# SamsungLabs/nb-asr

Hardware: AMD Instinct MI355X
Metric: utterances_per_sec (higher is better)
Workload: dtype f32

## Files before the change

### nb_asr_amd/csrc/grouped_conv.hip

```cpp
#include "grouped_conv_impl.h"

namespace nbasr {

__global__ __launch_bounds__(256) void pack_grouped_weights_kernel(const float* __restrict__ w, float* __restrict__ wp,
                                                                   int channels, int cg, int k)
{
    const int n = channels * cg * k;
    for (int i = blockIdx.x * blockDim.x + threadIdx.x; i < n; i += gridDim.x * blockDim.x) {
        int e = i;
        const int co = e % cg; e /= cg;
        const int j = e % k; e /= k;
        const int ci = e % cg; e /= cg;
        const int g = e;
        wp[i] = w[((static_cast<size_t>(g) * cg + co) * cg + ci) * k + j];
    }
}

constexpr int SF_QUADS = 32, SF_FRAMES = 4 * SF_QUADS, SF_LANES = 8, SF_MAX_PER_LANE = 16;
__global__ __launch_bounds__(SF_QUADS * SF_LANES) void stats_finalize_kernel(const float* __restrict__ part, float* __restrict__ stats,
                                                                               int batch, int frames, int ld, int groups, int cg, int gpp, float eps)
{
    __shared__ float s_cnt[SF_LANES][SF_FRAMES], s_mean[SF_LANES][SF_FRAMES], s_m2[SF_LANES][SF_FRAMES];
    const int tq = threadIdx.x & (SF_QUADS - 1), pl = threadIdx.x / SF_QUADS;
    const int t0 = blockIdx.x * SF_FRAMES + 4 * tq;
    const int b = blockIdx.y;
    const int nparts = (groups + gpp - 1) / gpp;
    float cnt[4] = {0.f, 0.f, 0.f, 0.f}, mean[4] = {0.f, 0.f, 0.f, 0.f}, m2[4] = {0.f, 0.f, 0.f, 0.f};
    if (t0 < frames) {
        float4 pm[SF_MAX_PER_LANE], pq[SF_MAX_PER_LANE];
#pragma unroll
        for (int u = 0; u < SF_MAX_PER_LANE; ++u) {
            const int k = pl + u * SF_LANES;
            pm[u] = make_float4(0.f, 0.f, 0.f, 0.f); pq[u] = pm[u];
            if (k < nparts) {
                const float* prow = part + (static_cast<size_t>(k) * batch + b) * 2 * ld + t0;
                pm[u] = *reinterpret_cast<const float4*>(prow);
                pq[u] = *reinterpret_cast<const float4*>(prow + ld);
            }
        }
#pragma unroll
        for (int u = 0; u < SF_MAX_PER_LANE; ++u) {
            const int k = pl + u * SF_LANES;
            if (k < nparts) {
                const float nb = static_cast<float>(cg * min(gpp, groups - gpp * k));
                const float pmv[4] = {pm[u].x, pm[u].y, pm[u].z, pm[u].w}, pqv[4] = {pq[u].x, pq[u].y, pq[u].z, pq[u].w};
#pragma unroll
                for (int r = 0; r < 4; ++r) {
                    const float tot = cnt[r] + nb;
                    const float delta = pmv[r] - mean[r];
                    mean[r] += delta * (nb / tot);
                    m2[r] += pqv[r] + delta * delta * (cnt[r] * nb / tot);
                    cnt[r] = tot;
                }
            }
        }
    }
#pragma unroll
    for (int r = 0; r < 4; ++r) { s_cnt[pl][4 * tq + r] = cnt[r]; s_mean[pl][4 * tq + r] = mean[r]; s_m2[pl][4 * tq + r] = m2[r]; }
    __syncthreads();
    const int tf = threadIdx.x, t = blockIdx.x * SF_FRAMES + tf;
    if (tf >= SF_FRAMES || t >= ld) return;
    float* srow = stats + static_cast<size_t>(b) * 2 * ld;
    if (t >= frames) { srow[t] = 0.f; srow[ld + t] = 0.f; return; }
    float c = s_cnt[0][tf], mu = s_mean[0][tf], q = s_m2[0][tf];
#pragma unroll
    for (int p = 1; p < SF_LANES; ++p) {
        const float nb = s_cnt[p][tf];
        if (nb > 0.f) {
            const float tot = c + nb;
            const float delta = s_mean[p][tf] - mu;
            mu += delta * (nb / tot);
            q += s_m2[p][tf] + delta * delta * (c * nb / tot);
            c = tot;
        }
    }
    srow[t] = mu;
    srow[ld + t] = 1.0f / sqrtf(q / c + eps);
}

template <typename T>
__global__ __launch_bounds__(256) void skip_sum_kernel(
    const T* __restrict__ s0, const T* __restrict__ s1, const T* __restrict__ s2,
    T* __restrict__ y, size_t nchunks, int channels, int nq, const LnRef ln_s0)
{
    constexpr int FR = Chunk<T>::FR;
    const size_t stride = static_cast<size_t>(gridDim.x) * blockDim.x;
    for (size_t i = static_cast<size_t>(blockIdx.x) * blockDim.x + threadIdx.x; i < nchunks; i += stride) {
        float o[FR];
#pragma unroll
        for (int e = 0; e < FR; ++e) o[e] = 0.f;
        if (s0) {
            float v[FR];
            load_frames<FR>(s0 + i * FR, v);
            if (ln_s0.stats) {
                const size_t row = i / nq;
                const int q = static_cast<int>(i - row * nq);
                const int c = static_cast<int>(row % channels);
                const size_t b = row / channels;
                const float* mrow = ln_s0.stats + b * 2 * (static_cast<size_t>(nq) * FR);
                float m[FR], r[FR];
                load_frames<FR>(mrow + q * FR, m);
                load_frames<FR>(mrow + static_cast<size_t>(nq) * FR + q * FR, r);
                const float gam = ln_s0.gamma[c], bet = ln_s0.beta[c];
#pragma unroll
                for (int e = 0; e < FR; ++e) v[e] = ln_apply(v[e], m[e], r[e], gam, bet);
            }
#pragma unroll
            for (int e = 0; e < FR; ++e) o[e] += v[e];
        }
        if (s1) {
            float v[FR];
            load_frames<FR>(s1 + i * FR, v);
#pragma unroll
            for (int e = 0; e < FR; ++e) o[e] += v[e];
        }
        if (s2) {
            float v[FR];
            load_frames<FR>(s2 + i * FR, v);
#pragma unroll
            for (int e = 0; e < FR; ++e) o[e] += v[e];
        }
        store_frames<FR, false>(y + i * FR, o);
    }
}

template <typename E>
__global__ __launch_bounds__(256) void repitch_kernel(
    const E* __restrict__ src, E* __restrict__ dst, int rows, int frames, int ld_src, int ld_dst)
{
    const int t = blockIdx.x * blockDim.x + threadIdx.x;
    if (t >= ld_dst) return;
    for (int r = blockIdx.y; r < rows; r += gridDim.y)
        dst[static_cast<size_t>(r) * ld_dst + t] = (t < frames) ? src[static_cast<size_t>(r) * ld_src + t] : E(0);
}

template <int CG, int K, int D, bool LNX, bool STATS>
__global__ __launch_bounds__(256) void grouped_conv_f32_kernel(
    const float* __restrict__ x, const float* __restrict__ w, const float* __restrict__ bias,
    const float* __restrict__ s0, const float* __restrict__ s1, const float* __restrict__ s2,
    float* __restrict__ y, int channels, int frames, int ld, int groups, const LnRef ln_x, const LnRef ln_s0,
    float* __restrict__ part)
{
    constexpr int LPAD = pad_left(K, D, 1);
    constexpr int SPAN = (K - 1) * D;
    constexpr int QL = (LPAD + 3) / 4;
    constexpr int QR = (SPAN - LPAD + 3) / 4;
    constexpr int NCH = QL + 1 + QR;
    constexpr int BASE = 4 * QL - LPAD;

    const int nq = ld >> 2;
    const int lane = threadIdx.x & 63;
    const int wave = threadIdx.x >> 6;
    const int q = blockIdx.x * 64 + lane;
    const int g = __builtin_amdgcn_readfirstlane(blockIdx.y * 4 + wave);
    const int b = blockIdx.z;
    if (!STATS && g >= groups) return;
    const bool active = q < nq && g < groups;

    const int ga = g < groups ? g : groups - 1;
    const size_t row0 = (static_cast<size_t>(b) * channels + static_cast<size_t>(ga) * CG) * ld;
    const float* __restrict__ wg = w + static_cast<size_t>(ga) * (CG * CG * K);
    const float* __restrict__ bg = bias + ga * CG;

    float acc[CG][4];
#pragma unroll
    for (int co = 0; co < CG; ++co) {
        const float bv = bg[co];
#pragma unroll
        for (int r = 0; r < 4; ++r) acc[co][r] = bv;
    }

    typedef float f2 __attribute__((ext_vector_type(2)));
    constexpr int NP = LNX ? NCH * 2 : 1;
    f2 nmw[NP], rw[NP], kw[NP];
    if (LNX) {
        const float4* __restrict__ mrow = reinterpret_cast<const float4*>(ln_x.stats + static_cast<size_t>(b) * 2 * ld);
        const float4* __restrict__ rrow = mrow + nq;
#pragma unroll
        for (int c = 0; c < NCH; ++c) {
            const int qq = q - QL + c;
            float4 m = make_float4(0.f, 0.f, 0.f, 0.f), r = m;
            if (active && qq >= 0 && qq < nq) { m = mrow[qq]; r = rrow[qq]; }
            nmw[(2 * c) % NP] = f2{-m.x, -m.y}; nmw[(2 * c + 1) % NP] = f2{-m.z, -m.w};
            rw[(2 * c) % NP] = f2{r.x, r.y};    rw[(2 * c + 1) % NP] = f2{r.z, r.w};
            kw[(2 * c) % NP] = f2{r.x != 0.f ? 1.f : 0.f, r.y != 0.f ? 1.f : 0.f};
            kw[(2 * c + 1) % NP] = f2{r.z != 0.f ? 1.f : 0.f, r.w != 0.f ? 1.f : 0.f};
        }
    }

#pragma unroll 1
    for (int ci = 0; ci < CG; ++ci) {
        const float4* __restrict__ xrow = reinterpret_cast<const float4*>(x + row0 + static_cast<size_t>(ci) * ld);
        float xw[NCH * 4];
#pragma unroll
        for (int c = 0; c < NCH; ++c) {
            const int qq = q - QL + c;
            float4 v = make_float4(0.f, 0.f, 0.f, 0.f);
            if (active && qq >= 0 && qq < nq) v = xrow[qq];
            xw[4 * c + 0] = v.x; xw[4 * c + 1] = v.y; xw[4 * c + 2] = v.z; xw[4 * c + 3] = v.w;
        }
        if (LNX) {
            const float gam = ln_x.gamma[ga * CG + ci], bet = ln_x.beta[ga * CG + ci];
            const f2 gam2 = f2{gam, gam}, bet2 = f2{bet, bet};
#pragma unroll
            for (int p = 0; p < NCH * 2; ++p) {
                f2 v = f2{xw[2 * p], xw[2 * p + 1]};
                v = (v + nmw[p % NP]) * rw[p % NP];
                v = __builtin_elementwise_fma(v, gam2, bet2) * kw[p % NP];
                xw[2 * p] = v.x; xw[2 * p + 1] = v.y;
            }
        }
#pragma unroll
        for (int j = 0; j < K; ++j) {
#pragma unroll
            for (int co = 0; co < CG; ++co) {
                const float wv = wg[(co * CG + ci) * K + j];
#pragma unroll
                for (int r = 0; r < 4; ++r)
                    acc[co][r] = __builtin_fmaf(wv, xw[BASE + r + j * D], acc[co][r]);
            }
        }
    }

    if (!STATS && !active) return;
    const int t0 = q * 4;
    const bool ragged = __any(active && t0 + 3 >= frames) != 0;
    float4 sm = make_float4(0.f, 0.f, 0.f, 0.f), sr = sm;
    if (active && s0 && ln_s0.stats) {
        const float4* __restrict__ mrow = reinterpret_cast<const float4*>(ln_s0.stats + static_cast<size_t>(b) * 2 * ld);
        sm = mrow[q];
        sr = mrow[nq + q];
    }
    if (active) {
#pragma unroll
    for (int co = 0; co < CG; ++co) {
        const size_t off = row0 + static_cast<size_t>(co) * ld + t0;
        float o[4];
#pragma unroll
        for (int r = 0; r < 4; ++r) o[r] = relu_clamp(acc[co][r]);
        if (s0) {
            float4 v = *reinterpret_cast<const float4*>(s0 + off);
            if (ln_s0.stats) {
                const float gam = ln_s0.gamma[ga * CG + co], bet = ln_s0.beta[ga * CG + co];
                v.x = ln_apply(v.x, sm.x, sr.x, gam, bet); v.y = ln_apply(v.y, sm.y, sr.y, gam, bet);
                v.z = ln_apply(v.z, sm.z, sr.z, gam, bet); v.w = ln_apply(v.w, sm.w, sr.w, gam, bet);
            }
            o[0] += v.x; o[1] += v.y; o[2] += v.z; o[3] += v.w;
        }
        if (s1) { const float4 v = *reinterpret_cast<const float4*>(s1 + off); o[0] += v.x; o[1] += v.y; o[2] += v.z; o[3] += v.w; }
        if (s2) { const float4 v = *reinterpret_cast<const float4*>(s2 + off); o[0] += v.x; o[1] += v.y; o[2] += v.z; o[3] += v.w; }
        if (ragged) {
#pragma unroll
            for (int r = 0; r < 4; ++r) if (t0 + r >= frames) o[r] = 0.f;
        }
        typedef float f4v __attribute__((ext_vector_type(4)));
        __builtin_nontemporal_store(f4v{o[0], o[1], o[2], o[3]}, reinterpret_cast<f4v*>(y + off));
        if (STATS) {
#pragma unroll
            for (int r = 0; r < 4; ++r) acc[co][r] = o[r];
        }
    }
    }
    if (STATS) {
        __shared__ float sp[4][8][64];
        float pm[4], p2[4];
#pragma unroll
        for (int r = 0; r < 4; ++r) {
            float sum = 0.f;
#pragma unroll
            for (int co = 0; co < CG; ++co) sum += acc[co][r];
            pm[r] = sum * (1.0f / CG);
            float m2 = 0.f;
#pragma unroll
            for (int co = 0; co < CG; ++co) { const float d = acc[co][r] - pm[r]; m2 = __builtin_fmaf(d, d, m2); }
            p2[r] = m2;
        }
#pragma unroll
        for (int r = 0; r < 4; ++r) { sp[wave][r][lane] = pm[r]; sp[wave][4 + r][lane] = p2[r]; }
        __syncthreads();
        if (wave == 0 && q < nq) {
            const int g0 = blockIdx.y * 4;
            const int nw = min(4, groups - g0);
            float om[4], o2[4];
#pragma unroll
            for (int r = 0; r < 4; ++r) {
                float mean = 0.f;
                for (int k = 0; k < nw; ++k) mean += sp[k][r][lane];
                mean /= static_cast<float>(nw);
                float m2 = 0.f;
                for (int k = 0; k < nw; ++k) { const float d = sp[k][r][lane] - mean; m2 += sp[k][4 + r][lane] + CG * d * d; }
                om[r] = mean; o2[r] = m2;
            }
            float* prow = part + (static_cast<size_t>(blockIdx.y) * gridDim.z + b) * 2 * ld + t0;
            *reinterpret_cast<float4*>(prow) = make_float4(om[0], om[1], om[2], om[3]);
            *reinterpret_cast<float4*>(prow + ld) = make_float4(o2[0], o2[1], o2[2], o2[3]);
        }
    }
}

template <int CG, int K, int D>
static int launch_grouped_f32(const GroupedArgs<float>& a, hipStream_t stream)
{
    const int nq = a.ld / 4;
    dim3 grid((nq + 63) / 64, (a.groups + 3) / 4, a.batch);
#define NBASR_LAUNCH_GROUPED(LNX, STATS)                                                                                  \
    hipLaunchKernelGGL((grouped_conv_f32_kernel<CG, K, D, LNX, STATS>), grid, dim3(256), 0, stream, a.x, a.w, a.bias, a.s0, a.s1, \
                       a.s2, a.y, a.channels, a.frames, a.ld, a.groups, a.ln_x, a.ln_s0, a.part)
    if (a.ln_x.stats) { if (a.part) NBASR_LAUNCH_GROUPED(true, true); else NBASR_LAUNCH_GROUPED(true, false); }
    else              { if (a.part) NBASR_LAUNCH_GROUPED(false, true); else NBASR_LAUNCH_GROUPED(false, false); }
#undef NBASR_LAUNCH_GROUPED
    return launch_status("nbasr_grouped_conv1d_node");
}

template <int CG>
static int dispatch_kd_f32(int kernel, int dilation, const GroupedArgs<float>& a, hipStream_t stream)
{
    if (kernel == 5 && dilation == 1) return launch_grouped_f32<CG, 5, 1>(a, stream);
    if (kernel == 5 && dilation == 2) return launch_grouped_f32<CG, 5, 2>(a, stream);
    if (kernel == 7 && dilation == 1) return launch_grouped_f32<CG, 7, 1>(a, stream);
    if (kernel == 7 && dilation == 2) return launch_grouped_f32<CG, 7, 2>(a, stream);
    set_error("nbasr_grouped_conv1d_node: unsupported (kernel=%d, dilation=%d); search space has k in {5,7}, d in {1,2}", kernel, dilation);
    return NBASR_EINVAL;
}

int grouped_conv_f32_base(const GroupedArgs<float>& a, int kernel, int dilation, hipStream_t stream)
{
    switch (a.channels / a.groups) {
        case 6:  return dispatch_kd_f32<6>(kernel, dilation, a, stream);
        case 8:  return dispatch_kd_f32<8>(kernel, dilation, a, stream);
        case 10: return dispatch_kd_f32<10>(kernel, dilation, a, stream);
        case 12: return dispatch_kd_f32<12>(kernel, dilation, a, stream);
        default:
            set_error("nbasr_grouped_conv1d_node: channels/groups=%d unsupported (model widths give 6, 8, 10, 12)", a.channels / a.groups);
            return NBASR_EINVAL;
    }
}

}

using namespace nbasr;

extern "C" size_t nbasr_grouped_stats_workspace_bytes(int batch, int ld, int groups)
{
    if (batch <= 0 || ld <= 0 || groups <= 0) return 0;
    return static_cast<size_t>(groups) * batch * 2 * ld * sizeof(float);
}

static int grouped_node_impl(const char* what, const void* x, const float* w, const float* bias, const void* skip0, const void* skip1,
                             const void* skip2, void* y, int batch, int channels, int frames, int ld, int groups, int kernel,
                             int dilation, const nbasr_deferred_ln* ln, int ln_on_x, int ln_on_skip0, float* stats_ws, int dtype,
                             int variant, nbasr_stream_t stream)
{
    NBASR_REQUIRE(dtype == NBASR_F32 || dtype == NBASR_BF16, NBASR_EINVAL, "%s: dtype %d is neither NBASR_F32 nor NBASR_BF16", what, dtype);
    const bool alt2 = variant > 0 && (variant & ~(NBASR_GC_OSPLIT | NBASR_GC_PIPE)) == 0;
    const bool ring = variant == NBASR_GC_RING;
    NBASR_REQUIRE((variant >= 0 && variant <= (NBASR_GC_FPL8 | NBASR_GC_WPERM)) || ((alt2 || ring) && dtype == NBASR_F32), NBASR_EINVAL,
                  "%s: unknown variant %d (NBASR_GC_OSPLIT / NBASR_GC_PIPE / NBASR_GC_RING: fp32 only, not with the other bits)", what, variant);
    NBASR_REQUIRE(aligned16(stats_ws), NBASR_EALIGN, "%s: statistics buffers must be 16-byte aligned", what);
    NBASR_REQUIRE(batch >= 0 && channels > 0 && frames >= 0 && groups > 0 && channels % groups == 0, NBASR_EINVAL,
                  "%s: bad sizes batch=%d channels=%d frames=%d groups=%d", what, batch, channels, frames, groups);
    if (batch == 0 || ld == 0) return NBASR_OK;
// ... 109 lines not shown
```

### nb_asr_amd/csrc/layernorm.hip

```cpp
#include "storage.h"

namespace nbasr {

constexpr int LN_ROWS = 16;
constexpr int LN_QS = 16;

template <typename T, bool MINMAX = false, int FR = Chunk<T>::FR>
__device__ __forceinline__ void tile_statistics(const T* x, int channels, int ld, float eps, size_t base, bool active,
                                                int row, int ql, float (*s_mean)[LN_QS * FR], float (*s_m2)[LN_QS * FR],
                                                float* s_cnt, float* s_mu, float* s_rstd,
                                                float (*s_lo)[LN_QS * FR] = nullptr, float (*s_hi)[LN_QS * FR] = nullptr)
{
    float shift[FR], s1[FR], s2[FR], lo[FR], hi[FR];
#pragma unroll
    for (int r = 0; r < FR; ++r) { shift[r] = 0.f; s1[r] = 0.f; s2[r] = 0.f; lo[r] = 3.0e38f; hi[r] = -3.0e38f; }
    int n = 0;
    if (active && row < channels) {
        load_frames<FR>(x + base + static_cast<size_t>(row) * ld, shift);
        auto fold = [&](const float (&e)[FR]) {
#pragma unroll
            for (int r = 0; r < FR; ++r) {
                const float d = e[r] - shift[r];
                s1[r] += d;
                s2[r] = __builtin_fmaf(d, d, s2[r]);
                if (MINMAX) { lo[r] = fminf(lo[r], e[r]); hi[r] = fmaxf(hi[r], e[r]); }
            }
            ++n;
        };
        int c = row;
        for (; c + 7 * LN_ROWS < channels; c += 8 * LN_ROWS) {
            float e[8][FR];
#pragma unroll
            for (int u = 0; u < 8; ++u) load_frames<FR>(x + base + static_cast<size_t>(c + u * LN_ROWS) * ld, e[u]);
#pragma unroll
            for (int u = 0; u < 8; ++u) fold(e[u]);
        }
        for (; c + 3 * LN_ROWS < channels; c += 4 * LN_ROWS) {
            float e[4][FR];
#pragma unroll
            for (int u = 0; u < 4; ++u) load_frames<FR>(x + base + static_cast<size_t>(c + u * LN_ROWS) * ld, e[u]);
#pragma unroll
            for (int u = 0; u < 4; ++u) fold(e[u]);
        }
        for (; c < channels; c += LN_ROWS) {
            float e[FR];
            load_frames<FR>(x + base + static_cast<size_t>(c) * ld, e);
            fold(e);
        }
    }
    const float fn = static_cast<float>(n);
#pragma unroll
    for (int r = 0; r < FR; ++r) {
        const float dm = n ? s1[r] / fn : 0.f;
        s_mean[row][ql * FR + r] = shift[r] + dm;
        s_m2[row][ql * FR + r] = n ? fmaxf(s2[r] - dm * s1[r], 0.f) : 0.f;
        if (MINMAX) { s_lo[row][ql * FR + r] = lo[r]; s_hi[row][ql * FR + r] = hi[r]; }
    }
    if (ql == 0) s_cnt[row] = fn;
    __syncthreads();

    if (threadIdx.x < LN_QS * FR) {
        const int col = threadIdx.x;
        float cnt = 0.f, mean = 0.f, m2 = 0.f;
#pragma unroll
        for (int k = 0; k < LN_ROWS; ++k) {
            const float nb = s_cnt[k];
            if (nb > 0.f) {
                const float tot = cnt + nb;
                const float delta = s_mean[k][col] - mean;
                mean += delta * (nb / tot);
                m2 += s_m2[k][col] + delta * delta * (cnt * nb / tot);
                cnt = tot;
            }
        }
        s_mu[col] = mean;
        s_rstd[col] = 1.0f / sqrtf(m2 / fmaxf(cnt, 1.f) + eps);
        if (MINMAX) {
            float l = s_lo[0][col], h = s_hi[0][col];
#pragma unroll
            for (int k = 1; k < LN_ROWS; ++k) { l = fminf(l, s_lo[k][col]); h = fmaxf(h, s_hi[k][col]); }
            s_lo[0][col] = l; s_hi[0][col] = h;
        }
    }
    __syncthreads();
}

template <typename TI, typename TO, bool ABSMAX>
__global__ __launch_bounds__(256) void layernorm_channels_kernel(
    const TI* x, const float* __restrict__ gamma, const float* __restrict__ beta,
    TO* y, int channels, int frames, int ld, float eps, unsigned* __restrict__ absmax)
{
    constexpr int FR = Chunk<TI>::FR;
    __shared__ float s_mean[LN_ROWS][LN_QS * FR];
    __shared__ float s_m2[LN_ROWS][LN_QS * FR];
    __shared__ float s_cnt[LN_ROWS];
    __shared__ float s_mu[LN_QS * FR];
    __shared__ float s_rstd[LN_QS * FR];

    const int ql = threadIdx.x & (LN_QS - 1);
    const int row = threadIdx.x / LN_QS;
    const int nq = ld / FR;
    const int q = blockIdx.x * LN_QS + ql;
    const int b = blockIdx.y;
    const bool active = q < nq;
    const size_t base = static_cast<size_t>(b) * channels * ld + static_cast<size_t>(q) * FR;

    tile_statistics<TI>(x, channels, ld, eps, base, active, row, ql, s_mean, s_m2, s_cnt, s_mu, s_rstd);

    if (!active && !ABSMAX) return;
    float mu[FR], rs[FR];
#pragma unroll
    for (int r = 0; r < FR; ++r) { mu[r] = s_mu[ql * FR + r]; rs[r] = s_rstd[ql * FR + r]; }
    const int t0 = q * FR;
    float amax = 0.f;
    for (int c = row; active && c < channels; c += LN_ROWS) {
        const size_t off = base + static_cast<size_t>(c) * ld;
        float o[FR];
        load_frames<FR>(x + off, o);
        const float g = gamma[c], bt = beta[c];
#pragma unroll
        for (int r = 0; r < FR; ++r) {
            o[r] = (o[r] - mu[r]) * rs[r] * g + bt;
            if (t0 + r >= frames) o[r] = 0.f;
            if (ABSMAX) amax = fmaxf(amax, finite_abs(o[r]));
        }
        store_frames<FR, false>(y + off, o);
    }
    if (ABSMAX) {
#pragma unroll
        for (int m = 32; m >= 1; m >>= 1) amax = fmaxf(amax, __shfl_xor(amax, m));
        if ((threadIdx.x & 63) == 0) atomicMax(absmax + b, __float_as_uint(amax));
    }
}

template <typename T>
__global__ __launch_bounds__(256) void channel_stats_kernel(const T* __restrict__ x, float* __restrict__ stats,
                                                            int channels, int frames, int ld, float eps)
{
    constexpr int FR = Chunk<T>::FR;
    __shared__ float s_mean[LN_ROWS][LN_QS * FR];
    __shared__ float s_m2[LN_ROWS][LN_QS * FR];
    __shared__ float s_cnt[LN_ROWS];
    __shared__ float s_mu[LN_QS * FR];
    __shared__ float s_rstd[LN_QS * FR];

    const int ql = threadIdx.x & (LN_QS - 1);
    const int row = threadIdx.x / LN_QS;
    const int nq = ld / FR;
    const int q = blockIdx.x * LN_QS + ql;
    const int b = blockIdx.y;
    const bool active = q < nq;
    const size_t base = static_cast<size_t>(b) * channels * ld + static_cast<size_t>(q) * FR;

    tile_statistics<T>(x, channels, ld, eps, base, active, row, ql, s_mean, s_m2, s_cnt, s_mu, s_rstd);

    if (threadIdx.x < LN_QS * FR) {
        const int t = blockIdx.x * (LN_QS * FR) + threadIdx.x;
        if (t < ld) {
            const bool live = t < frames;
            float* srow = stats + static_cast<size_t>(b) * 2 * ld;
            srow[t] = live ? s_mu[threadIdx.x] : 0.f;
            srow[ld + t] = live ? s_rstd[threadIdx.x] : 0.f;
        }
    }
}

}

using namespace nbasr;

static int layernorm_impl(const char* what, const void* x, const float* gamma, const float* beta, void* y, float* absmax,
                          int batch, int channels, int frames, int ld, float eps, nbasr_stream_t stream,
                          int in_dtype = NBASR_F32, int out_dtype = NBASR_F32)
{
    clear_error();
    NBASR_REQUIRE((in_dtype == NBASR_F32 || in_dtype == NBASR_BF16) && (out_dtype == NBASR_F32 || out_dtype == NBASR_BF16) &&
                  !(in_dtype == NBASR_F32 && out_dtype == NBASR_BF16), NBASR_EINVAL,
                  "%s: storage types (%d -> %d) unsupported (f32 -> f32, bf16 -> bf16, bf16 -> f32)", what, in_dtype, out_dtype);
    NBASR_REQUIRE(batch >= 0 && channels > 0 && frames >= 0, NBASR_EINVAL, "%s: bad sizes", what);
    const int fr = in_dtype == NBASR_BF16 ? 8 : 4;
    NBASR_REQUIRE(ld >= frames && ld % fr == 0, NBASR_EALIGN, "%s: ld=%d must be >= frames=%d and a multiple of %d", what, ld, frames, fr);
    if (batch == 0 || ld == 0) return NBASR_OK;
    NBASR_REQUIRE(x && gamma && beta && y, NBASR_ENULL, "%s: NULL pointer", what);
    NBASR_REQUIRE(aligned16(x) && aligned16(y), NBASR_EALIGN, "%s: x, y must be 16-byte aligned", what);
    NBASR_REQUIRE(batch <= 65535, NBASR_EINVAL, "%s: batch %d > 65535", what, batch);
    NBASR_REQUIRE(!absmax || in_dtype == NBASR_F32, NBASR_EINVAL, "%s: the absmax by-product exists for fp32 tensors only", what);
    const int nq = ld / fr;
    const dim3 grid((nq + LN_QS - 1) / LN_QS, batch);
    if (in_dtype == NBASR_BF16) {
        if (out_dtype == NBASR_BF16)
            hipLaunchKernelGGL((layernorm_channels_kernel<bf16_t, bf16_t, false>), grid, dim3(256), 0, as_stream(stream),
                               static_cast<const bf16_t*>(x), gamma, beta, static_cast<bf16_t*>(y), channels, frames, ld, eps, static_cast<unsigned*>(nullptr));
        else
            hipLaunchKernelGGL((layernorm_channels_kernel<bf16_t, float, false>), grid, dim3(256), 0, as_stream(stream),
                               static_cast<const bf16_t*>(x), gamma, beta, static_cast<float*>(y), channels, frames, ld, eps, static_cast<unsigned*>(nullptr));
    } else if (absmax) {
        zero_async(absmax, sizeof(float) * batch, as_stream(stream));
        hipLaunchKernelGGL((layernorm_channels_kernel<float, float, true>), grid, dim3(256), 0, as_stream(stream),
                           static_cast<const float*>(x), gamma, beta, static_cast<float*>(y), channels, frames, ld, eps, reinterpret_cast<unsigned*>(absmax));
    } else {
        hipLaunchKernelGGL((layernorm_channels_kernel<float, float, false>), grid, dim3(256), 0, as_stream(stream),
                           static_cast<const float*>(x), gamma, beta, static_cast<float*>(y), channels, frames, ld, eps, static_cast<unsigned*>(nullptr));
    }
    return launch_status(what);
}

extern "C" int nbasr_layernorm_channels(const void* x, const float* gamma, const float* beta, void* y, float* absmax, int batch,
                                        int channels, int frames, int ld, float eps, int in_dtype, int out_dtype, nbasr_stream_t stream)
{
    clear_error();
    NBASR_REQUIRE(!absmax || (in_dtype == NBASR_F32 && out_dtype == NBASR_F32), NBASR_EINVAL,
                  "nbasr_layernorm_channels: the max|y| by-product exists for fp32 -> fp32 only");
    return layernorm_impl("nbasr_layernorm_channels", x, gamma, beta, y, absmax, batch, channels, frames, ld, eps, stream, in_dtype, out_dtype);
}

__global__ __launch_bounds__(256) void channel_stats_bound_kernel(const float* __restrict__ x, const float* __restrict__ gamma,
                                                                  const float* __restrict__ beta, float* __restrict__ stats,
                                                                  unsigned* __restrict__ bound, int channels, int frames, int ld, float eps)
{
    __shared__ float s_mean[LN_ROWS][LN_QS * 4];
    __shared__ float s_m2[LN_ROWS][LN_QS * 4];
    __shared__ float s_cnt[LN_ROWS];
    __shared__ float s_mu[LN_QS * 4];
    __shared__ float s_rstd[LN_QS * 4];
    __shared__ float s_gb[8];
    __shared__ float s_lo[LN_ROWS][LN_QS * 4];
    __shared__ float s_hi[LN_ROWS][LN_QS * 4];

    const int ql = threadIdx.x & (LN_QS - 1);
    const int row = threadIdx.x / LN_QS;
    const int nq = ld >> 2;
    const int q = blockIdx.x * LN_QS + ql;
    const int b = blockIdx.y;
    const bool active = q < nq;
    const size_t base = static_cast<size_t>(b) * channels * ld + static_cast<size_t>(q) * 4;

    float gm = 0.f, bm = 0.f;
    for (int c = threadIdx.x; c < channels; c += 256) { gm = fmaxf(gm, fabsf(gamma[c])); bm = fmaxf(bm, fabsf(beta[c])); }
#pragma unroll
    for (int d = 32; d >= 1; d >>= 1) { gm = fmaxf(gm, __shfl_xor(gm, d)); bm = fmaxf(bm, __shfl_xor(bm, d)); }
    if ((threadIdx.x & 63) == 0) { s_gb[threadIdx.x >> 6] = gm; s_gb[4 + (threadIdx.x >> 6)] = bm; }

    tile_statistics<float, true>(x, channels, ld, eps, base, active, row, ql, s_mean, s_m2, s_cnt, s_mu, s_rstd, s_lo, s_hi);
    gm = fmaxf(fmaxf(s_gb[0], s_gb[1]), fmaxf(s_gb[2], s_gb[3]));
    bm = fmaxf(fmaxf(s_gb[4], s_gb[5]), fmaxf(s_gb[6], s_gb[7]));

    float dev = 0.f;
    if (threadIdx.x < LN_QS * 4) {
        const int t = blockIdx.x * (LN_QS * 4) + threadIdx.x;
        if (t < ld) {
            const bool live = t < frames;
            float* srow = stats + static_cast<size_t>(b) * 2 * ld;
            srow[t] = live ? s_mu[threadIdx.x] : 0.f;
            srow[ld + t] = live ? s_rstd[threadIdx.x] : 0.f;
            if (live) dev = finite_abs(fmaxf(s_hi[0][threadIdx.x] - s_mu[threadIdx.x], s_mu[threadIdx.x] - s_lo[0][threadIdx.x]) * s_rstd[threadIdx.x]);
        }
    }
    if (threadIdx.x < 64) {
#pragma unroll
        for (int d = 32; d >= 1; d >>= 1) dev = fmaxf(dev, __shfl_xor(dev, d));
        if (threadIdx.x == 0) atomicMax(bound + b, __float_as_uint(finite_abs((dev * gm + bm) * 1.0001f)));
    }
}

template <bool NORM>
__global__ __launch_bounds__(256) void normalize_split_kernel(const float* __restrict__ x, const float* __restrict__ stats,
                                                              const float* __restrict__ gamma, const float* __restrict__ beta,
                                                              const float* __restrict__ bound, unsigned char* __restrict__ image,
                                                              int channels, int , int ld,
                                                              int bound_stride)
{
    typedef _Float16 halfx8 __attribute__((ext_vector_type(8)));
    constexpr int SPLIT_PITCH = 68;
    __shared__ __attribute__((aligned(16))) unsigned char s_tile[4][2][4 * SPLIT_PITCH * 16];
    const int ql = threadIdx.x & 63, wv = threadIdx.x >> 6, oct0 = wv + 4 * blockIdx.z;
    const int nq = ld >> 2;
    const int q = blockIdx.x * 64 + ql;
    const int b = blockIdx.y;
    const int n_groups = (channels + 15) >> 4;
    const size_t rows = static_cast<size_t>(ld) + 1;
    unsigned char* const img_b = image + static_cast<size_t>(b) * n_groups * 4 * rows * 16;
    if (blockIdx.x == 0 && blockIdx.z == 0) {
        const uint4 z = make_uint4(0u, 0u, 0u, 0u);
        for (int pl = threadIdx.x; pl < n_groups * 4; pl += 256) *reinterpret_cast<uint4*>(img_b + static_cast<size_t>(pl) * rows * 16) = z;
    }
    if (blockIdx.x * 64 >= nq) return;
    const bool inside = q < nq;
    float scale = 1.f;
    {
        const unsigned bits = __float_as_uint(bound[static_cast<size_t>(b) * bound_stride]);
        const int e = static_cast<int>((bits >> 23) & 0xffu);
        int k = (bits & 0x7fffffffu) ? (127 + 14) - e : 0;
        k = k > 126 ? 126 : (k < -126 ? -126 : k);
        scale = __uint_as_float(static_cast<unsigned>(127 + k) << 23);
    }
    float m4[4] = {0.f, 0.f, 0.f, 0.f}, r4[4] = {0.f, 0.f, 0.f, 0.f};
    if constexpr (NORM) {
        if (inside) {
            const float* st = stats + static_cast<size_t>(b) * 2 * ld + q * 4;
            const float4 mu = *reinterpret_cast<const float4*>(st), rs = *reinterpret_cast<const float4*>(st + ld);
            m4[0] = mu.x; m4[1] = mu.y; m4[2] = mu.z; m4[3] = mu.w;
            r4[0] = rs.x; r4[1] = rs.y; r4[2] = rs.z; r4[3] = rs.w;
        }
    }
    const float* xb = x + static_cast<size_t>(b) * channels * ld + static_cast<size_t>(q) * 4;
    const int n_oct = (channels + 7) >> 3;
    const int oct_step = 4 * gridDim.z;
    auto load_octet = [&](int oct, float4 (&t)[8]) {
#pragma unroll
        for (int c = 0; c < 8; ++c) {
            const int ch = oct * 8 + c;
            t[c] = make_float4(0.f, 0.f, 0.f, 0.f);
            if (inside && oct < n_oct && ch < channels) t[c] = *reinterpret_cast<const float4*>(xb + static_cast<size_t>(ch) * ld);
        }
    };
    unsigned char* const tile_hi = s_tile[wv][0];
    unsigned char* const tile_lo = s_tile[wv][1];
    float4 cur[8];
    if (oct0 < 2 * n_groups) load_octet(oct0, cur);
    for (int oct = oct0; oct < 2 * n_groups; oct += oct_step) {
        float4 nxt[8];
        if (oct + oct_step < 2 * n_groups) load_octet(oct + oct_step, nxt);
        else {
#pragma unroll
            for (int c = 0; c < 8; ++c) nxt[c] = make_float4(0.f, 0.f, 0.f, 0.f);
        }
        float v[8][4];
#pragma unroll
        for (int c = 0; c < 8; ++c) {
            const int ch = oct * 8 + c;
            float g = 0.f, be = 0.f;
            if constexpr (NORM) {
                if (oct < n_oct && ch < channels) { g = gamma[ch]; be = beta[ch]; }
            }
            const float e4[4] = {cur[c].x, cur[c].y, cur[c].z, cur[c].w};
#pragma unroll
            for (int r = 0; r < 4; ++r) {
                if constexpr (NORM) v[c][r] = (ch < channels) ? ln_apply(e4[r], m4[r], r4[r], g, be) * scale : 0.f;
                else                v[c][r] = e4[r] * scale;
            }
        }
#pragma unroll
        for (int r = 0; r < 4; ++r) {
            halfx8 hi, lo;
#pragma unroll
            for (int c = 0; c < 8; ++c) {
                const _Float16 h = static_cast<_Float16>(v[c][r]);
                hi[c] = h;
                lo[c] = static_cast<_Float16>(v[c][r] - static_cast<float>(h));
            }
            *reinterpret_cast<halfx8*>(tile_hi + (r * SPLIT_PITCH + ql) * 16) = hi;
            *reinterpret_cast<halfx8*>(tile_lo + (r * SPLIT_PITCH + ql) * 16) = lo;
        }
        asm volatile("s_waitcnt lgkmcnt(0)" ::: "memory");
        unsigned char* plane_hi = img_b + ((static_cast<size_t>(oct >> 1) * 4 + (oct & 1)) * rows + 1 + static_cast<size_t>(blockIdx.x) * 256) * 16;
        unsigned char* plane_lo = plane_hi + 2 * rows * 16;
#pragma unroll
        for (int k = 0; k < 4; ++k) {
            const int src = ((ql & 3) * SPLIT_PITCH + 16 * k + (ql >> 2)) * 16;
            const halfx8 hi = *reinterpret_cast<const halfx8*>(tile_hi + src);
            const halfx8 lo = *reinterpret_cast<const halfx8*>(tile_lo + src);
            const int f = 64 * k + ql;
            if (blockIdx.x * 256 + f < ld) {
                *reinterpret_cast<halfx8*>(plane_hi + f * 16) = hi;
                *reinterpret_cast<halfx8*>(plane_lo + f * 16) = lo;
            }
        }
        asm volatile("s_waitcnt lgkmcnt(0)" ::: "memory");
#pragma unroll
        for (int c = 0; c < 8; ++c) cur[c] = nxt[c];
    }
}

static int split_grid_z(int tiles, int batch)
{
    const long long wgs = static_cast<long long>(tiles) * batch;
    int z = 4;
    while (z < 16 && wgs * z < 512) z *= 2;
    return z;
}

extern "C" int nbasr_layernorm_split_image(const float* x, const float* gamma, const float* beta, float* stats, float* bound,
                                           void* image, int batch, int channels, int frames, int ld, float eps,
                                           nbasr_stream_t stream)
{
    clear_error();
    NBASR_REQUIRE(batch >= 0 && channels > 0 && frames >= 0, NBASR_EINVAL, "nbasr_layernorm_split_image: bad sizes");
    NBASR_REQUIRE(ld >= frames && ld % 4 == 0, NBASR_EALIGN, "nbasr_layernorm_split_image: ld=%d must be >= frames=%d and a multiple of 4", ld, frames);
    if (batch == 0 || ld == 0) return NBASR_OK;
    NBASR_REQUIRE(x && gamma && beta && stats && bound && image, NBASR_ENULL, "nbasr_layernorm_split_image: NULL pointer");
    NBASR_REQUIRE(aligned16(x) && aligned16(stats) && aligned16(image), NBASR_EALIGN, "nbasr_layernorm_split_image: x, stats, image must be 16-byte aligned");
    NBASR_REQUIRE(batch <= 65535, NBASR_EINVAL, "nbasr_layernorm_split_image: batch %d > 65535", batch);
    zero_async(bound, sizeof(float) * batch, as_stream(stream));
    const int nq = ld / 4;
    hipLaunchKernelGGL(channel_stats_bound_kernel, dim3((nq + LN_QS - 1) / LN_QS, batch), dim3(256), 0, as_stream(stream),
                       x, gamma, beta, stats, reinterpret_cast<unsigned*>(bound), channels, frames, ld, eps);
    hipLaunchKernelGGL(normalize_split_kernel<true>, dim3((nq + 63) / 64, batch, split_grid_z((nq + 63) / 64, batch)), dim3(256), 0, as_stream(stream),
                       x, stats, gamma, beta, bound, static_cast<unsigned char*>(image), channels, frames, ld, 1);
    return launch_status("nbasr_layernorm_split_image");
}

__global__ __launch_bounds__(256) void input_range_kernel(const float* __restrict__ x, unsigned* __restrict__ range,
                                                          int channels, int frames, int ld)
{
    __shared__ float s_max[4][256];
    __shared__ unsigned s_bad[4];
    const int b = blockIdx.y;
    const int lane = threadIdx.x & 63, slice = threadIdx.x >> 6;
    const int t0 = (blockIdx.x * 64 + lane) * 4;
    float m[4] = {0.f, 0.f, 0.f, 0.f};
    unsigned bad = 0u;
    if (t0 < frames) {
        const float* col = x + static_cast<size_t>(b) * channels * ld + t0;
        const bool whole = t0 + 4 <= ld && ld % 4 == 0 && (reinterpret_cast<size_t>(x) & 15) == 0;
        for (int c = slice; c < channels; c += 4) {
            float v[4] = {0.f, 0.f, 0.f, 0.f};
            if (whole) {
                const float4 q = *reinterpret_cast<const float4*>(col + static_cast<size_t>(c) * ld);
                v[0] = q.x; v[1] = q.y; v[2] = q.z; v[3] = q.w;
            } else {
#pragma unroll
                for (int r = 0; r < 4; ++r) if (t0 + r < frames) v[r] = col[static_cast<size_t>(c) * ld + r];
            }
#pragma unroll
            for (int r = 0; r < 4; ++r) {
                const float a = fabsf(v[r]);
                if (t0 + r < frames) {
                    if (!(a <= 3.4028234664e38f)) bad = 1u;
                    else m[r] = fmaxf(m[r], a);
                }
            }
        }
    }
#pragma unroll
    for (int r = 0; r < 4; ++r) s_max[slice][lane * 4 + r] = m[r];
#pragma unroll
    for (int d = 32; d >= 1; d >>= 1) bad |= __shfl_xor(bad, d);
    if (lane == 0) s_bad[slice] = bad;
    __syncthreads();
    const int t = blockIdx.x * 256 + threadIdx.x;
    const float fmax_ = fmaxf(fmaxf(s_max[0][threadIdx.x], s_max[1][threadIdx.x]), fmaxf(s_max[2][threadIdx.x], s_max[3][threadIdx.x]));
    float hi = fmax_, lo = (t < frames && fmax_ > 0.f) ? fmax_ : __uint_as_float(0x7f800000u);
#pragma unroll
    for (int d = 32; d >= 1; d >>= 1) {
        hi = fmaxf(hi, __shfl_xor(hi, d));
        lo = fminf(lo, __shfl_xor(lo, d));
    }
    if (lane == 0) {
        atomicMax(range + 4 * b, __float_as_uint(hi));
        atomicMin(range + 4 * b + 1, __float_as_uint(lo));
        if (slice == 0 && (s_bad[0] | s_bad[1] | s_bad[2] | s_bad[3])) atomicOr(range + 4 * b + 2, 0x3f800000u);
    }
}

__global__ void input_range_init_kernel(unsigned* __restrict__ range, int batch)
{
    const int b = blockIdx.x * blockDim.x + threadIdx.x;
    if (b < batch) { range[4 * b] = 0u; range[4 * b + 1] = 0x7f800000u; range[4 * b + 2] = 0u; range[4 * b + 3] = 0u; }
}

extern "C" int nbasr_input_range(const float* x, float* range, int batch, int channels, int frames, int ld, nbasr_stream_t stream)
{
    clear_error();
    NBASR_REQUIRE(batch >= 0 && channels > 0 && frames >= 0 && ld >= frames, NBASR_EINVAL, "nbasr_input_range: bad sizes");
    if (batch == 0) return NBASR_OK;
    NBASR_REQUIRE(range, NBASR_ENULL, "nbasr_input_range: range is NULL");
    NBASR_REQUIRE(batch <= 65535, NBASR_EINVAL, "nbasr_input_range: batch %d > 65535", batch);
    hipLaunchKernelGGL(input_range_init_kernel, dim3((batch + 255) / 256), dim3(256), 0, as_stream(stream), reinterpret_cast<unsigned*>(range), batch);
    if (frames > 0) {
        NBASR_REQUIRE(x, NBASR_ENULL, "nbasr_input_range: x is NULL");
        hipLaunchKernelGGL(input_range_kernel, dim3((frames + 255) / 256, batch), dim3(256), 0, as_stream(stream), x,
                           reinterpret_cast<unsigned*>(range), channels, frames, ld);
    }
    return launch_status("nbasr_input_range");
}

extern "C" int nbasr_split_image_ranged(const float* x, const float* x_range, void* image, int batch, int channels, int frames,
                                        int ld, nbasr_stream_t stream)
{
    clear_error();
    NBASR_REQUIRE(batch >= 0 && channels > 0 && frames >= 0, NBASR_EINVAL, "nbasr_split_image_ranged: bad sizes");
    NBASR_REQUIRE(ld >= frames && ld % 4 == 0, NBASR_EALIGN, "nbasr_split_image_ranged: ld=%d must be >= frames=%d and a multiple of 4", ld, frames);
    if (batch == 0 || ld == 0) return NBASR_OK;
    NBASR_REQUIRE(x && x_range && image, NBASR_ENULL, "nbasr_split_image_ranged: NULL pointer");
    NBASR_REQUIRE(aligned16(x) && aligned16(image), NBASR_EALIGN, "nbasr_split_image_ranged: x, image must be 16-byte aligned");
    NBASR_REQUIRE(batch <= 65535, NBASR_EINVAL, "nbasr_split_image_ranged: batch %d > 65535", batch);
    const int nq = ld / 4;
    hipLaunchKernelGGL(normalize_split_kernel<false>, dim3((nq + 63) / 64, batch, split_grid_z((nq + 63) / 64, batch)), dim3(256), 0, as_stream(stream),
                       x, static_cast<const float*>(nullptr), static_cast<const float*>(nullptr), static_cast<const float*>(nullptr),
                       x_range, static_cast<unsigned char*>(image), channels, frames, ld, 4);
    return launch_status("nbasr_split_image_ranged");
}

extern "C" int nbasr_channel_stats(const void* x, float* stats, int batch, int channels, int frames, int ld, float eps, int dtype,
                                     nbasr_stream_t stream)
{
    clear_error();
    NBASR_REQUIRE(dtype == NBASR_F32 || dtype == NBASR_BF16, NBASR_EINVAL, "nbasr_channel_stats: unknown dtype %d", dtype);
    NBASR_REQUIRE(batch >= 0 && channels > 0 && frames >= 0, NBASR_EINVAL, "nbasr_channel_stats: bad sizes");
    const int fr = dtype == NBASR_BF16 ? 8 : 4;
    NBASR_REQUIRE(ld >= frames && ld % fr == 0, NBASR_EALIGN, "nbasr_channel_stats: ld=%d must be >= frames=%d and a multiple of %d", ld, frames, fr);
    if (batch == 0 || ld == 0) return NBASR_OK;
    NBASR_REQUIRE(x && stats, NBASR_ENULL, "nbasr_channel_stats: NULL pointer");
    NBASR_REQUIRE(aligned16(x) && aligned16(stats), NBASR_EALIGN, "nbasr_channel_stats: x, stats must be 16-byte aligned");
    NBASR_REQUIRE(batch <= 65535, NBASR_EINVAL, "nbasr_channel_stats: batch %d > 65535", batch);
    const int nq = ld / fr;
    const dim3 grid((nq + LN_QS - 1) / LN_QS, batch);
    if (dtype == NBASR_BF16)
        hipLaunchKernelGGL(channel_stats_kernel<bf16_t>, grid, dim3(256), 0, as_stream(stream), static_cast<const bf16_t*>(x), stats, channels, frames, ld, eps);
    else
        hipLaunchKernelGGL(channel_stats_kernel<float>, grid, dim3(256), 0, as_stream(stream), static_cast<const float*>(x), stats, channels, frames, ld, eps);
    return launch_status("nbasr_channel_stats");
}

template <typename T, bool NORM>
__global__ __launch_bounds__(256) void bf16_image_kernel(const T* __restrict__ x, const float* __restrict__ stats,
                                                         const float* __restrict__ gamma, const float* __restrict__ beta,
                                                         unsigned char* __restrict__ image, int channels, int frames, int ld)
{
    constexpr int FR = Chunk<T>::FR;
    const int ql = threadIdx.x & 15, oct0 = threadIdx.x >> 4;
    const int nq = ld / FR;
    const int q = blockIdx.x * 16 + ql;
    const int b = blockIdx.y;
    const int n_groups = (channels + 15) >> 4;
    const size_t rows = static_cast<size_t>(ld) + 1;
    unsigned char* const img_b = image + static_cast<size_t>(b) * n_groups * 2 * rows * 16;
    if (blockIdx.x == 0) {
        const uint4 z = make_uint4(0u, 0u, 0u, 0u);
        for (int pl = threadIdx.x; pl < n_groups * 2; pl += 256) *reinterpret_cast<uint4*>(img_b + static_cast<size_t>(pl) * rows * 16) = z;
    }
    if (q >= nq) return;
    float m[FR], r[FR];
#pragma unroll
    for (int e = 0; e < FR; ++e) { m[e] = 0.f; r[e] = 1.f; }
    if (NORM) {
        const float* st = stats + static_cast<size_t>(b) * 2 * ld + q * FR;
        load_frames<FR>(st, m);
        load_frames<FR>(st + ld, r);
    }
    const T* xb = x + static_cast<size_t>(b) * channels * ld + static_cast<size_t>(q) * FR;
    const int n_oct = (channels + 7) >> 3;
    for (int oct = oct0; oct < 2 * n_groups; oct += 16) {
        float v[8][FR];
#pragma unroll
        for (int c = 0; c < 8; ++c) {
            const int ch = oct * 8 + c;
#pragma unroll
            for (int e = 0; e < FR; ++e) v[c][e] = 0.f;
            if (oct < n_oct && ch < channels) {
                load_frames<FR>(xb + static_cast<size_t>(ch) * ld, v[c]);
                if (NORM) {
                    const float g = gamma[ch], be = beta[ch];
#pragma unroll
                    for (int e = 0; e < FR; ++e) v[c][e] = ln_apply(v[c][e], m[e], r[e], g, be);
                } else {
#pragma unroll
                    for (int e = 0; e < FR; ++e) if (q * FR + e >= frames) v[c][e] = 0.f;
                }
            }
        }
        unsigned char* plane = img_b + ((static_cast<size_t>(oct >> 1) * 2 + (oct & 1)) * rows + 1 + static_cast<size_t>(q) * FR) * 16;
#pragma unroll
        for (int e = 0; e < FR; ++e) {
            const u4v row = {pack_bf16x2(v[0][e], v[1][e]), pack_bf16x2(v[2][e], v[3][e]), pack_bf16x2(v[4][e], v[5][e]), pack_bf16x2(v[6][e], v[7][e])};
            *reinterpret_cast<u4v*>(plane + e * 16) = row;
        }
    }
}

extern "C" size_t nbasr_bf16_image_bytes(int batch, int channels, int ld)
{
    if (batch <= 0 || channels <= 0 || ld < 0) return 0;
    return static_cast<size_t>(batch) * ((channels + 15) / 16) * 2 * (static_cast<size_t>(ld) + 1) * 16;
}

extern "C" int nbasr_bf16_image(const void* x, const float* gamma, const float* beta, float* stats, void* image, int batch,
                                int channels, int frames, int ld, float eps, int dtype, nbasr_stream_t stream)
{
    clear_error();
    NBASR_REQUIRE(dtype == NBASR_F32 || dtype == NBASR_BF16, NBASR_EINVAL, "nbasr_bf16_image: unknown dtype %d", dtype);
    NBASR_REQUIRE(batch >= 0 && channels > 0 && frames >= 0, NBASR_EINVAL, "nbasr_bf16_image: bad sizes");
    const int fr = dtype == NBASR_BF16 ? 8 : 4;
    NBASR_REQUIRE(ld >= frames && ld % fr == 0, NBASR_EALIGN, "nbasr_bf16_image: ld=%d must be >= frames=%d and a multiple of %d", ld, frames, fr);
    if (batch == 0 || ld == 0) return NBASR_OK;
    NBASR_REQUIRE(x && image, NBASR_ENULL, "nbasr_bf16_image: NULL pointer");
    const bool norm = gamma != nullptr;
    NBASR_REQUIRE(!norm || (beta && stats), NBASR_ENULL, "nbasr_bf16_image: LayerNorm needs gamma, beta and the stats buffer");
    NBASR_REQUIRE(aligned16(x) && aligned16(stats) && aligned16(image), NBASR_EALIGN, "nbasr_bf16_image: x, stats, image must be 16-byte aligned");
    NBASR_REQUIRE(batch <= 65535, NBASR_EINVAL, "nbasr_bf16_image: batch %d > 65535", batch);
    const int nq = ld / fr;
    if (norm) {
        const int rc = nbasr_channel_stats(x, stats, batch, channels, frames, ld, eps, dtype, stream);
        if (rc != NBASR_OK) return rc;
    }
    const dim3 grid((nq + 15) / 16, batch);
    unsigned char* img = static_cast<unsigned char*>(image);
#define NBASR_IMG(T, NORM) hipLaunchKernelGGL((bf16_image_kernel<T, NORM>), grid, dim3(256), 0, as_stream(stream), static_cast<const T*>(x), \
                                              stats, gamma, beta, img, channels, frames, ld)
    if (dtype == NBASR_BF16) { if (norm) NBASR_IMG(bf16_t, true); else NBASR_IMG(bf16_t, false); }
    else                     { if (norm) NBASR_IMG(float, true); else NBASR_IMG(float, false); }
#undef NBASR_IMG
    return launch_status("nbasr_bf16_image");
}

template <typename TI, typename TO>
__global__ __launch_bounds__(256) void convert_kernel(const TI* __restrict__ x, TO* __restrict__ y, size_t n8)
{
    for (size_t i = static_cast<size_t>(blockIdx.x) * blockDim.x + threadIdx.x; i < n8; i += static_cast<size_t>(gridDim.x) * blockDim.x) {
        float v[8];
        load_frames<8>(x + i * 8, v);
        store_frames<8, false>(y + i * 8, v);
    }
}

extern "C" int nbasr_convert(const void* x, void* y, long long n, int in_dtype, int out_dtype, nbasr_stream_t stream)
{
    clear_error();
    NBASR_REQUIRE(n >= 0 && n % 8 == 0, NBASR_EINVAL, "nbasr_convert: n=%lld must be a non-negative multiple of 8", n);
    NBASR_REQUIRE((in_dtype == NBASR_F32 && out_dtype == NBASR_BF16) || (in_dtype == NBASR_BF16 && out_dtype == NBASR_F32), NBASR_EINVAL,
                  "nbasr_convert: conversions are f32 -> bf16 and bf16 -> f32");
    if (n == 0) return NBASR_OK;
    NBASR_REQUIRE(x && y, NBASR_ENULL, "nbasr_convert: NULL pointer");
    NBASR_REQUIRE(aligned16(x) && aligned16(y), NBASR_EALIGN, "nbasr_convert: pointers must be 16-byte aligned");
    const size_t n8 = static_cast<size_t>(n / 8);
    const unsigned blocks = static_cast<unsigned>(n8 / 256 + 1 < 8192 ? n8 / 256 + 1 : 8192);
    if (in_dtype == NBASR_F32)
        hipLaunchKernelGGL((convert_kernel<float, bf16_t>), dim3(blocks), dim3(256), 0, as_stream(stream), static_cast<const float*>(x), static_cast<bf16_t*>(y), n8);
    else
        hipLaunchKernelGGL((convert_kernel<bf16_t, float>), dim3(blocks), dim3(256), 0, as_stream(stream), static_cast<const bf16_t*>(x), static_cast<float*>(y), n8);
    return launch_status("nbasr_convert");
}
```

Before: 11250.

## Widen stats-bound blocks to 1024 threads and simplify partial-stat merging

```diff
diff --git a/nb_asr_amd/csrc/grouped_conv.hip b/nb_asr_amd/csrc/grouped_conv.hip
--- a/nb_asr_amd/csrc/grouped_conv.hip
+++ b/nb_asr_amd/csrc/grouped_conv.hip
@@ -25,7 +25,7 @@
     const int t0 = blockIdx.x * SF_FRAMES + 4 * tq;
     const int b = blockIdx.y;
     const int nparts = (groups + gpp - 1) / gpp;
-    float cnt[4] = {0.f, 0.f, 0.f, 0.f}, mean[4] = {0.f, 0.f, 0.f, 0.f}, m2[4] = {0.f, 0.f, 0.f, 0.f};
+    float cnt = 0.f, mean[4] = {0.f, 0.f, 0.f, 0.f}, m2[4] = {0.f, 0.f, 0.f, 0.f};
     if (t0 < frames) {
         float4 pm[SF_MAX_PER_LANE], pq[SF_MAX_PER_LANE];
 #pragma unroll
@@ -44,19 +44,20 @@
             if (k < nparts) {
                 const float nb = static_cast<float>(cg * min(gpp, groups - gpp * k));
                 const float pmv[4] = {pm[u].x, pm[u].y, pm[u].z, pm[u].w}, pqv[4] = {pq[u].x, pq[u].y, pq[u].z, pq[u].w};
+                const float tot = cnt + nb;
+                const float wm = nb / tot, wq = cnt * nb / tot;
 #pragma unroll
                 for (int r = 0; r < 4; ++r) {
-                    const float tot = cnt[r] + nb;
                     const float delta = pmv[r] - mean[r];
-                    mean[r] += delta * (nb / tot);
-                    m2[r] += pqv[r] + delta * delta * (cnt[r] * nb / tot);
-                    cnt[r] = tot;
+                    mean[r] += delta * wm;
+                    m2[r] += pqv[r] + delta * delta * wq;
                 }
-            }
-        }
-    }
-#pragma unroll
-    for (int r = 0; r < 4; ++r) { s_cnt[pl][4 * tq + r] = cnt[r]; s_mean[pl][4 * tq + r] = mean[r]; s_m2[pl][4 * tq + r] = m2[r]; }
+                cnt = tot;
+            }
+        }
+    }
+#pragma unroll
+    for (int r = 0; r < 4; ++r) { s_cnt[pl][4 * tq + r] = cnt; s_mean[pl][4 * tq + r] = mean[r]; s_m2[pl][4 * tq + r] = m2[r]; }
     __syncthreads();
     const int tf = threadIdx.x, t = blockIdx.x * SF_FRAMES + tf;
     if (tf >= SF_FRAMES || t >= ld) return;
diff --git a/nb_asr_amd/csrc/layernorm.hip b/nb_asr_amd/csrc/layernorm.hip
--- a/nb_asr_amd/csrc/layernorm.hip
+++ b/nb_asr_amd/csrc/layernorm.hip
@@ -5,11 +5,11 @@
 constexpr int LN_ROWS = 16;
 constexpr int LN_QS = 16;
 
-template <typename T, bool MINMAX = false, int FR = Chunk<T>::FR>
+template <typename T, bool MINMAX = false, int QS = LN_QS, int FR = Chunk<T>::FR>
 __device__ __forceinline__ void tile_statistics(const T* x, int channels, int ld, float eps, size_t base, bool active,
-                                                int row, int ql, float (*s_mean)[LN_QS * FR], float (*s_m2)[LN_QS * FR],
+                                                int row, int ql, float (*s_mean)[QS * FR], float (*s_m2)[QS * FR],
                                                 float* s_cnt, float* s_mu, float* s_rstd,
-                                                float (*s_lo)[LN_QS * FR] = nullptr, float (*s_hi)[LN_QS * FR] = nullptr)
+                                                float (*s_lo)[QS * FR] = nullptr, float (*s_hi)[QS * FR] = nullptr)
 {
     float shift[FR], s1[FR], s2[FR], lo[FR], hi[FR];
 #pragma unroll
@@ -35,17 +35,14 @@
 #pragma unroll
             for (int u = 0; u < 8; ++u) fold(e[u]);
         }
-        for (; c + 3 * LN_ROWS < channels; c += 4 * LN_ROWS) {
-            float e[4][FR];
-#pragma unroll
-            for (int u = 0; u < 4; ++u) load_frames<FR>(x + base + static_cast<size_t>(c + u * LN_ROWS) * ld, e[u]);
-#pragma unroll
-            for (int u = 0; u < 4; ++u) fold(e[u]);
-        }
-        for (; c < channels; c += LN_ROWS) {
-            float e[FR];
-            load_frames<FR>(x + base + static_cast<size_t>(c) * ld, e);
-            fold(e);
+        if (c < channels) {
+            float e[7][FR];
+#pragma unroll
+            for (int u = 0; u < 7; ++u)
+                if (c + u * LN_ROWS < channels) load_frames<FR>(x + base + static_cast<size_t>(c + u * LN_ROWS) * ld, e[u]);
+#pragma unroll
+            for (int u = 0; u < 7; ++u)
+                if (c + u * LN_ROWS < channels) fold(e[u]);
         }
     }
     const float fn = static_cast<float>(n);
@@ -59,7 +56,7 @@
     if (ql == 0) s_cnt[row] = fn;
     __syncthreads();
 
-    if (threadIdx.x < LN_QS * FR) {
+    if (threadIdx.x < QS * FR) {
         const int col = threadIdx.x;
         float cnt = 0.f, mean = 0.f, m2 = 0.f;
 #pragma unroll
@@ -214,52 +211,57 @@
     return layernorm_impl("nbasr_layernorm_channels", x, gamma, beta, y, absmax, batch, channels, frames, ld, eps, stream, in_dtype, out_dtype);
 }
 
-__global__ __launch_bounds__(256) void channel_stats_bound_kernel(const float* __restrict__ x, const float* __restrict__ gamma,
-                                                                  const float* __restrict__ beta, float* __restrict__ stats,
-                                                                  unsigned* __restrict__ bound, int channels, int frames, int ld, float eps)
-{
-    __shared__ float s_mean[LN_ROWS][LN_QS * 4];
-    __shared__ float s_m2[LN_ROWS][LN_QS * 4];
+constexpr int SB_QS = 64, SB_COLS = SB_QS * 4, SB_THREADS = LN_ROWS * SB_QS;
+__global__ __launch_bounds__(SB_THREADS) void channel_stats_bound_kernel(const float* __restrict__ x, const float* __restrict__ gamma,
+                                                                         const float* __restrict__ beta, float* __restrict__ stats,
+                                                                         unsigned* __restrict__ bound, int channels, int frames, int ld, float eps)
+{
+    __shared__ float s_mean[LN_ROWS][SB_COLS];
+    __shared__ float s_m2[LN_ROWS][SB_COLS];
     __shared__ float s_cnt[LN_ROWS];
-    __shared__ float s_mu[LN_QS * 4];
-    __shared__ float s_rstd[LN_QS * 4];
-    __shared__ float s_gb[8];
-    __shared__ float s_lo[LN_ROWS][LN_QS * 4];
-    __shared__ float s_hi[LN_ROWS][LN_QS * 4];
-
-    const int ql = threadIdx.x & (LN_QS - 1);
-    const int row = threadIdx.x / LN_QS;
+    __shared__ float s_mu[SB_COLS];
+    __shared__ float s_rstd[SB_COLS];
+    __shared__ float s_gb[2 * LN_ROWS];
+    __shared__ float s_lo[LN_ROWS][SB_COLS];
+    __shared__ float s_hi[LN_ROWS][SB_COLS];
+
+    const int ql = threadIdx.x & (SB_QS - 1);
+    const int row = threadIdx.x / SB_QS;
     const int nq = ld >> 2;
-    const int q = blockIdx.x * LN_QS + ql;
+    const int q = blockIdx.x * SB_QS + ql;
     const int b = blockIdx.y;
     const bool active = q < nq;
     const size_t base = static_cast<size_t>(b) * channels * ld + static_cast<size_t>(q) * 4;
 
-    float gm = 0.f, bm = 0.f;
-    for (int c = threadIdx.x; c < channels; c += 256) { gm = fmaxf(gm, fabsf(gamma[c])); bm = fmaxf(bm, fabsf(beta[c])); }
+    const int c0 = min(static_cast<int>(threadIdx.x), channels - 1);
+    const float g0 = gamma[c0], b0 = beta[c0];
+
+    tile_statistics<float, true, SB_QS>(x, channels, ld, eps, base, active, row, ql, s_mean, s_m2, s_cnt, s_mu, s_rstd, s_lo, s_hi);
+
+    float gm = fmaxf(0.f, fabsf(g0)), bm = fmaxf(0.f, fabsf(b0));
+    for (int c = threadIdx.x + SB_THREADS; c < channels; c += SB_THREADS) { gm = fmaxf(gm, fabsf(gamma[c])); bm = fmaxf(bm, fabsf(beta[c])); }
 #pragma unroll
     for (int d = 32; d >= 1; d >>= 1) { gm = fmaxf(gm, __shfl_xor(gm, d)); bm = fmaxf(bm, __shfl_xor(bm, d)); }
-    if ((threadIdx.x & 63) == 0) { s_gb[threadIdx.x >> 6] = gm; s_gb[4 + (threadIdx.x >> 6)] = bm; }
-
-    tile_statistics<float, true>(x, channels, ld, eps, base, active, row, ql, s_mean, s_m2, s_cnt, s_mu, s_rstd, s_lo, s_hi);
-    gm = fmaxf(fmaxf(s_gb[0], s_gb[1]), fmaxf(s_gb[2], s_gb[3]));
-    bm = fmaxf(fmaxf(s_gb[4], s_gb[5]), fmaxf(s_gb[6], s_gb[7]));
-
+    if (ql == 0) { s_gb[row] = gm; s_gb[LN_ROWS + row] = bm; }
+    __syncthreads();
+    if (threadIdx.x >= SB_COLS) return;
+
+    const int t = blockIdx.x * SB_COLS + threadIdx.x;
     float dev = 0.f;
-    if (threadIdx.x < LN_QS * 4) {
-        const int t = blockIdx.x * (LN_QS * 4) + threadIdx.x;
-        if (t < ld) {
-            const bool live = t < frames;
-            float* srow = stats + static_cast<size_t>(b) * 2 * ld;
-            srow[t] = live ? s_mu[threadIdx.x] : 0.f;
-            srow[ld + t] = live ? s_rstd[threadIdx.x] : 0.f;
-            if (live) dev = finite_abs(fmaxf(s_hi[0][threadIdx.x] - s_mu[threadIdx.x], s_mu[threadIdx.x] - s_lo[0][threadIdx.x]) * s_rstd[threadIdx.x]);
-        }
-    }
-    if (threadIdx.x < 64) {
-#pragma unroll
-        for (int d = 32; d >= 1; d >>= 1) dev = fmaxf(dev, __shfl_xor(dev, d));
-        if (threadIdx.x == 0) atomicMax(bound + b, __float_as_uint(finite_abs((dev * gm + bm) * 1.0001f)));
+    if (t < ld) {
+        const bool live = t < frames;
+        float* srow = stats + static_cast<size_t>(b) * 2 * ld;
+        srow[t] = live ? s_mu[threadIdx.x] : 0.f;
+        srow[ld + t] = live ? s_rstd[threadIdx.x] : 0.f;
+        if (live) dev = finite_abs(fmaxf(s_hi[0][threadIdx.x] - s_mu[threadIdx.x], s_mu[threadIdx.x] - s_lo[0][threadIdx.x]) * s_rstd[threadIdx.x]);
+    }
+#pragma unroll
+    for (int d = 32; d >= 1; d >>= 1) dev = fmaxf(dev, __shfl_xor(dev, d));
+    if (ql == 0 && t < ld) {
+        gm = s_gb[0]; bm = s_gb[LN_ROWS];
+#pragma unroll
+        for (int k = 1; k < LN_ROWS; ++k) { gm = fmaxf(gm, s_gb[k]); bm = fmaxf(bm, s_gb[LN_ROWS + k]); }
+        atomicMax(bound + b, __float_as_uint(finite_abs((dev * gm + bm) * 1.0001f)));
     }
 }
 
@@ -393,7 +395,7 @@
     NBASR_REQUIRE(batch <= 65535, NBASR_EINVAL, "nbasr_layernorm_split_image: batch %d > 65535", batch);
     zero_async(bound, sizeof(float) * batch, as_stream(stream));
     const int nq = ld / 4;
-    hipLaunchKernelGGL(channel_stats_bound_kernel, dim3((nq + LN_QS - 1) / LN_QS, batch), dim3(256), 0, as_stream(stream),
+    hipLaunchKernelGGL(channel_stats_bound_kernel, dim3((nq + SB_QS - 1) / SB_QS, batch), dim3(SB_THREADS), 0, as_stream(stream),
                        x, gamma, beta, stats, reinterpret_cast<unsigned*>(bound), channels, frames, ld, eps);
     hipLaunchKernelGGL(normalize_split_kernel<true>, dim3((nq + 63) / 64, batch, split_grid_z((nq + 63) / 64, batch)), dim3(256), 0, as_stream(stream),
                        x, stats, gamma, beta, bound, static_cast<unsigned char*>(image), channels, frames, ld, 1);
```

Result: no change. 11300 (median of 6 runs) (+0.4%).
